# xcompact3d/x3d2

Measured on AMD Instinct MI355X. Metric: DoF*steps/s (whole node), TGV 512^3 per GPU, full fractional step, higher is better.
Workload: dtype f64; 1 GPU; TGV 512x512x512 all-periodic, Re=1600, dt=1e-3, RK3 (3 substeps/step), compact6/classic schemes, rocFFT Poisson (configs[2]); per_gpu=512^3, driver=fused, parallelism=domain decomposition 1x1x1, decomposition=yslabs, decomposition_requested=auto, poisson_z_first=228

## Files before the change

include/x3d2_hip.h:

```cpp
#ifndef X3D2_HIP_H
#define X3D2_HIP_H

#include <stddef.h>

#ifdef X3D_SINGLE_PREC
typedef float x3d_real;
#else
typedef double x3d_real;
#endif

#ifdef __cplusplus
extern "C" {
#endif

enum { X3D_DIR_X = 1, X3D_DIR_Y = 2, X3D_DIR_Z = 3, X3D_DIR_C = 4 };
enum { X3D_BC_PERIODIC = 0, X3D_BC_NEUMANN = 1, X3D_BC_DIRICHLET = 2, X3D_BC_HALO = -1 };
enum { X3D_X_FACE = 1100, X3D_Y_FACE = 1010, X3D_Z_FACE = 110 };
#define X3D_N_HALO 4

typedef struct x3d_backend x3d_backend;
typedef struct x3d_tdsops x3d_tdsops;
typedef struct x3d_poisson x3d_poisson;

const char *x3d_last_error(void);
// ... 231 lines not shown
int x3d_sfft010_set_waves(x3d_sfft010 *p, const x3d_real *waves, const x3d_real *ax, const x3d_real *bx, const x3d_real *ay,
                          const x3d_real *by, const x3d_real *az, const x3d_real *bz);
int x3d_sfft010_set_stretching(x3d_sfft010 *p, int sym, const x3d_real *a0, const x3d_real *a1);
int x3d_sfft010_periodicity_y(x3d_sfft010 *p, x3d_real *f_out, const x3d_real *f_in, int undo);
int x3d_sfft010_forward_local(x3d_sfft010 *p, const x3d_real *f_in, x3d_real *sendbuf);
int x3d_sfft010_fft_z(x3d_sfft010 *p, x3d_real *recvbuf, int dir);
int x3d_sfft010_postprocess_010(x3d_sfft010 *p, x3d_real *recvbuf);
int x3d_sfft010_backward_local(x3d_sfft010 *p, const x3d_real *sendbuf, x3d_real *f_out);

int x3d_poisson_zfirst_ok(x3d_poisson *p, int *ok);
int x3d_tds_pair_zfirst_ok(x3d_backend *b, const x3d_tdsops *ta, const x3d_tdsops *tb, int *ok);
int x3d_poisson_zfirst_middle(x3d_poisson *p);
int x3d_poisson_zfirst_forward(x3d_poisson *p, const x3d_real *f_in);
int x3d_poisson_zfirst_backward(x3d_poisson *p, x3d_real *f_out);
int x3d_poisson_solve_000_zfirst(x3d_poisson *p, x3d_real *f);
int x3d_poisson_set_stretching_zfirst(x3d_poisson *p, int sym, const x3d_real *a0, const x3d_real *a1);
int x3d_poisson_create_proxy(x3d_backend *b, x3d_poisson **out, x3d_real *spectrum, int ny, long px, int (*middle)(void *user),
                             void *user);
int x3d_poisson_solve_010_rows_zfirst(x3d_poisson *p, x3d_real *f);
int x3d_tds_pair_zfirst(x3d_backend *b, x3d_poisson *poisson, int mode, x3d_real *out1, x3d_real *out2, const x3d_real *in1,
                        const x3d_real *in2, const x3d_tdsops *ta, const x3d_tdsops *tb, int *done);

typedef struct x3d_sfftz x3d_sfftz;
int x3d_sfftz_create(x3d_backend *b, x3d_sfftz **out, const int nglob_cell[3], int py, int ry, int parts);
int x3d_sfftz_destroy(x3d_sfftz *p);
int x3d_sfftz_sizes(const x3d_sfftz *p, long out[16]);
int x3d_sfftz_spectrum(const x3d_sfftz *p, x3d_real **c, int *ny, long *px);
int x3d_sfftz_set_waves(x3d_sfftz *p, const x3d_real *rw, const x3d_real *ax, const x3d_real *bx, const x3d_real *ay,
                        const x3d_real *by, const x3d_real *az, const x3d_real *bz);
int x3d_sfftz_tds_pair(x3d_sfftz *p, int mode, x3d_real *out1, x3d_real *out2, const x3d_real *in1, const x3d_real *in2,
// ... 166 lines not shown
```

x3d2_amd/_lib.py:

```python
import ctypes
import os
import subprocess

from .common import X3dError

HERE = os.path.dirname(os.path.abspath(__file__))
SINGLE = os.environ.get("X3D_SINGLE_PREC") == "1"
LIB_PATH = os.path.join(HERE, "libx3d2_hip_sp.so" if SINGLE else "libx3d2_hip.so")
CSRC = os.path.join(HERE, "csrc")

REAL = ctypes.c_float if SINGLE else ctypes.c_double
NP_REAL = "float32" if SINGLE else "float64"
c_double_p = ctypes.POINTER(REAL)
c_int_p = ctypes.POINTER(ctypes.c_int)
VP = ctypes.c_void_p
I, D, SZT = ctypes.c_int, REAL, ctypes.c_size_t


def torch_real():
    import torch
    return torch.float32 if SINGLE else torch.float64

PROTOTYPES = {
    "x3d_last_error": (ctypes.c_char_p, []),
# ... 141 lines not shown
    "x3d_sfft010_postprocess_010_part": (I, [VP, VP, I]),
    "x3d_sfft010_destroy": (I, [VP]),
    "x3d_sfft010_sizes": (I, [VP, ctypes.POINTER(ctypes.c_long)]),
    "x3d_sfft010_set_waves": (I, [VP] + [c_double_p] * 7),
    "x3d_sfft010_set_stretching": (I, [VP, I, c_double_p, c_double_p]),
    "x3d_sfft010_periodicity_y": (I, [VP, VP, VP, I]),
    "x3d_sfft010_forward_local": (I, [VP, VP, VP]),
    "x3d_sfft010_fft_z": (I, [VP, VP, I]),
    "x3d_sfft010_postprocess_010": (I, [VP, VP]),
    "x3d_sfft010_backward_local": (I, [VP, VP, VP]),
    "x3d_poisson_zfirst_ok": (I, [VP, c_int_p]),
    "x3d_poisson_zfirst_middle": (I, [VP]),
    "x3d_poisson_zfirst_forward": (I, [VP, VP]),
    "x3d_poisson_zfirst_backward": (I, [VP, VP]),
    "x3d_poisson_solve_000_zfirst": (I, [VP, VP]),
    "x3d_tds_pair_zfirst": (I, [VP, VP, I, VP, VP, VP, VP, VP, VP, c_int_p]),
    "x3d_sfftz_create": (I, [VP, ctypes.POINTER(VP), c_int_p, I, I, I]),
    "x3d_sfftz_destroy": (I, [VP]),
    "x3d_sfftz_sizes": (I, [VP, ctypes.POINTER(ctypes.c_long)]),
    "x3d_sfftz_set_waves": (I, [VP] + [c_double_p] * 7),
    "x3d_sfftz_tds_pair": (I, [VP, I, VP, VP, VP, VP, VP, VP, c_int_p]),
    "x3d_sfftz_z": (I, [VP, VP, I]),
    "x3d_sfftz_z_field": (I, [VP, VP, I]),
    "x3d_sfftz_x_forward": (I, [VP, VP, I]),
    "x3d_sfftz_y_stage": (I, [VP, VP, I, I]),
    "x3d_sfftz_x_backward": (I, [VP, VP, I]),
    "x3d_sfftz_tds_pair_rows": (I, [VP, I, VP, VP, VP, VP, VP, VP, I, I, c_int_p]),
    "x3d_sfftz_z_rows": (I, [VP, VP, I, I, I]),
    "x3d_sfftz_x_forward_rows": (I, [VP, VP, I, I, I]),
    "x3d_sfftz_x_backward_rows": (I, [VP, VP, I, I, I]),
# ... 134 lines not shown
```

x3d2_amd/backend.py:

```python
import ctypes

import numpy as np
import torch

from . import _lib
from .common import (CELL, DIR_C, DIR_X, DIR_Y, DIR_Z, N_HALO, NULL_LOC, VERT, X_FACE, Y_FACE, Z_FACE, X3dError,
                     get_rdr_from_dirs, move_data_loc)
from .field import Allocator
from .parallel import Comm
from .switches import Switches
from .tdsops import Tdsops

VP = ctypes.c_void_p


def _dp(a):
    if a.dtype != np.dtype(_lib.NP_REAL):
        a = np.ascontiguousarray(a, dtype=_lib.NP_REAL)
    return a.ctypes.data_as(_lib.c_double_p)


class HipBackend:
    n_halo = N_HALO

# ... 615 lines not shown

    def zfirst_pairs_ok(self, t_a, t_b):
        flag = ctypes.c_int(0)
        _lib.check(self.lib.x3d_tds_pair_zfirst_ok(self.h, t_a.handle, t_b.handle, ctypes.byref(flag)))
        return bool(flag.value)

    def tds_apply_mean(self, du, u, tdsops, direction, mean_target):
        if u.data_loc == NULL_LOC:
            raise X3dError("You must set the data_loc before calling volume integral.")
        out = VP()
        ncell = float(np.prod(self.mesh.get_global_dims(CELL)))
        _lib.check(self.lib.x3d_tds_solve_mean(self.h, du.ptr, u.ptr, tdsops.handle, direction, self._dims(u.data_loc), ncell,
                                               float(mean_target), ctypes.byref(out)))
        return out

    def tds_apply(self, du, u, tdsops, direction, accumulate=False, scale=1.0):
        if not self._decomposed(direction):
            _lib.check(self.lib.x3d_tds_solve_acc(self.h, du.ptr, u.ptr, tdsops.handle, direction,
                                                  int(accumulate), float(scale)))
            return
        self._tds_dist(du, u, tdsops, direction, accumulate=accumulate, scale=scale)

    def tds_solve(self, du, u, tdsops):
        if u.dir != du.dir:
            raise X3dError("DIR mismatch between fields in tds_solve.")
        if u.data_loc != NULL_LOC:
            du.set_data_loc(move_data_loc(u.data_loc, u.dir, tdsops.move))
        direction = u.dir
        if direction == DIR_C:
            raise X3dError("tds_solve needs a directional field")
# ... 460 lines not shown
```

x3d2_amd/csrc/common.h:

```cpp
#pragma once
#include <hip/hip_runtime.h>

#include <cstdarg>
#include <cstdio>
#include <cstring>
#include <vector>

#include "../../include/x3d2_hip.h"

typedef x3d_real real_t;
#ifdef X3D_SINGLE_PREC
typedef float2 real2_t;
#define make_real2 make_float2
#else
typedef double2 real2_t;
#define make_real2 make_double2
#endif
#ifdef X3D_SINGLE_PREC
#define X3D_FFT_R2C HIPFFT_R2C
#define X3D_FFT_C2R HIPFFT_C2R
#define X3D_FFT_C2C HIPFFT_C2C
#define x3d_fftExecR2C hipfftExecR2C
#define x3d_fftExecC2R hipfftExecC2R
#define x3d_fftExecC2C hipfftExecC2C
// ... 70 lines not shown
    z = (z ^ (z >> 30)) * 0xBF58476D1CE4E5B9ull;
    z = (z ^ (z >> 27)) * 0x94D049BB133111EBull;
    return z ^ (z >> 31);
}

struct PencilGeom {
    int np;
    int dim0;
    long s0, s1, rs;
};

#define X3D_SW_UNSET (-0x7fffffffL - 1)
struct x3d_switches {
    long no_via_x, no_xscan, no_ygen, no_ytile, no_q5, no_direct, sfft010_split_xy;
    long no_circ, no_halo_circ, no_uniform, xscan_p1, no_ztile, no_tds_pair, no_npw2, no_tile3, xdir_generic, no_xcirc;
    long no_tds_lincomb, no_zfirst010, no_zfirst, no_xwide, no_xwide_upd;
    long no_spectral_pad, no_fft512, no_rwt, no_r2c512, no_y010, y010_no_db, no_onchip2, no_slab_fused_z;
    long lazy_dump, lazy_report, lazy_keep_zero_terms;
    long pad_x;
    long slab_z_split;
    long lazy_rules;
    long y010_form;
    long via_x;
    long ytile;
    long ygen;
    long x_fast;
    long x_tq3;
    long x_circ;
};
void x3d_switches_from_env(x3d_switches *sw);

// ... 213 lines not shown
```

x3d2_amd/csrc/poisson.hip:

```cpp
#include "fft_util.h"
#include "poisson_priv.h"
#include "spectral000.h"
int x3d_proxy_hook(x3d_poisson *p, int which, real_t *f);

__global__ void k_fill_pad(real_t *__restrict__ a, size_t rows, int nxm, int nxs, real_t v)
{
    const size_t r = (size_t)blockIdx.x * blockDim.x + threadIdx.x;
    if (r >= rows) return;
    for (int i = nxm; i < nxs; i++) a[r * nxs + i] = v;
}

static int upload_pitched(void *dst, const void *src, size_t rows, int nxm, int nxs, size_t elem)
{
    X3D_HIP(hipMemset(dst, 0, rows * nxs * elem));
    X3D_HIP(hipMemcpy2D(dst, nxs * elem, src, nxm * elem, nxm * elem, rows, hipMemcpyHostToDevice));
    return 0;
}

__global__ void __launch_bounds__(256)
    k_process_spectral_000(real2_t *__restrict__ c, const real_t *__restrict__ waves, int nxs, int ny, int nz,
                           int nx, const real_t *__restrict__ ax, const real_t *__restrict__ bx,
                           const real_t *__restrict__ ay, const real_t *__restrict__ by,
                           const real_t *__restrict__ az, const real_t *__restrict__ bz)
{
// ... 77 lines not shown
        p->r2c512 = p->nx == 512 && (batch % 2) == 0 && !b->sw.no_r2c512;
    }
    *out = p;
    return 0;
}

extern "C" int x3d_poisson_destroy(x3d_poisson *p)
{
    X3D_RANGE(__func__);
    if (!p) return 0;
    if (p->ext_middle) { delete p; return 0; }
    hipfftDestroy(p->plan_fw);
    hipfftDestroy(p->plan_bw);
    if (p->fast512) { hipfftDestroy(p->plan_x_fw); hipfftDestroy(p->plan_x_bw); }
    if (p->y010 == 1) { hipfftDestroy(p->plan_x010_fw); hipfftDestroy(p->plan_x010_bw); }
    hipFree(p->c); hipFree(p->waves); hipFree(p->ab); hipFree(p->work); hipFree(p->rwT); hipFree(p->rwZ);
    hipFree(p->lu[0]); hipFree(p->lu[1]); hipFree(p->luz[0]); hipFree(p->luz[1]);
    delete p;
    return 0;
}

static int x_forward_512(x3d_poisson *p, const real_t *f)
{
    ProfScope ps(p->b, X3D_K_FFT, 1);
    if (p->r2c512)
        return x3d_fft512_r2c(p->b, (real2_t *)p->c, f, (long)p->ny * p->nz, p->b->nxp, p->nxs);
    X3D_FFT(hipfftSetStream(p->plan_x_fw, p->b->stream));
    X3D_FFT(x3d_fftExecR2C(p->plan_x_fw, (x3d_fft_real *)f, (x3d_fft_cplx *)p->c));
    return 0;
}

// ... 422 lines not shown
```

x3d2_amd/csrc/poisson_priv.h:

```cpp
#pragma once
#include <hipfft/hipfft.h>

#include "common.h"

struct x3d_poisson {
    x3d_backend *b;
    int nx, ny, nz;
    int nxm, nxs;
    hipfftHandle plan_fw, plan_bw;
    real2_t *c;
    real_t *waves;
    real_t *rwT;
    real_t *ab;
    void *work;
    size_t work_size;
    int stretched, sym;
    real_t *lu[2];
    real_t *luz[2];
    size_t c_elems;
    int fast512;
    int r2c512;
    hipfftHandle plan_x_fw, plan_x_bw;
    int y010;
    hipfftHandle plan_x010_fw, plan_x010_bw;
    real_t *rwZ;
    int (*ext_middle)(void *user);
    void *ext_user;
    real2_t *ext_c;
    int ext_ny;
    long ext_px;
};
```

x3d2_amd/csrc/switches.hip:

```cpp
#include <cstdlib>

#include "common.h"

enum SwKind {
    SW_FLAG,
    SW_INT,
    SW_MASK,
    SW_FORM,
};
struct SwEntry {
    const char *name;
    SwKind kind;
    long unset;
    long x3d_switches::*field;
};
#define F(name, field) {name, SW_FLAG, 0, &x3d_switches::field}
static const SwEntry g_table[] = {
    F("X3D_NO_XSCAN", no_xscan),
    F("X3D_XDIR_GENERIC", xdir_generic),
    F("X3D_XSCAN_P1", xscan_p1),
    F("X3D_NO_TILE3", no_tile3),
    F("X3D_NO_XCIRC", no_xcirc),
    F("X3D_NO_CIRC", no_circ),
    F("X3D_NO_HALO_CIRC", no_halo_circ),
// ... 3 lines not shown
    F("X3D_NO_XWIDE_UPD", no_xwide_upd),
    F("X3D_NO_VIA_X", no_via_x),
    F("X3D_NO_YTILE", no_ytile),
    F("X3D_NO_ZTILE", no_ztile),
    F("X3D_NO_YGEN", no_ygen),
    F("X3D_NO_Q5", no_q5),
    F("X3D_NO_DIRECT", no_direct),
    F("X3D_NO_TDS_PAIR", no_tds_pair),
    F("X3D_NO_NPW2", no_npw2),
    F("X3D_NO_ONCHIP2", no_onchip2),
    F("X3D_NO_SPECTRAL_PAD", no_spectral_pad),
    F("X3D_NO_FFT512", no_fft512),
    F("X3D_NO_RWT", no_rwt),
    F("X3D_NO_R2C512", no_r2c512),
    F("X3D_NO_ZFIRST", no_zfirst),
    F("X3D_NO_ZFIRST010", no_zfirst010),
    F("X3D_NO_Y010", no_y010),
    F("X3D_Y010_NO_DB", y010_no_db),
    F("X3D_SFFT010_SPLIT_XY", sfft010_split_xy),
    F("X3D_NO_SLAB_FUSED_Z", no_slab_fused_z),
    F("X3D_LAZY_DUMP", lazy_dump),
    F("X3D_LAZY_REPORT", lazy_report),
    F("X3D_LAZY_KEEP_ZERO_TERMS", lazy_keep_zero_terms),
    {"X3D_LAZY_RULES", SW_MASK, 0xffffffffL, &x3d_switches::lazy_rules},
    {"X3D_PAD_X", SW_INT, X3D_SW_UNSET, &x3d_switches::pad_x},
    {"X3D_SLAB_Z_SPLIT", SW_INT, -1, &x3d_switches::slab_z_split},
    {"X3D_Y010_FORM", SW_FORM, 1, &x3d_switches::y010_form},
};
#undef F

// ... 34 lines not shown
```

x3d2_amd/csrc/tds.hip:

```cpp
#include "common.h"
#include "zfft_tile.h"

extern "C" int x3d_tdsops_create(x3d_backend *b, x3d_tdsops **out, int n_tds, int n_rhs, int move,
                                 int periodic, const real_t *coeffs, const real_t *coeffs_s,
                                 const real_t *coeffs_e, const real_t *dist_fw, const real_t *dist_bw,
                                 const real_t *dist_sa, const real_t *dist_sc, const real_t *dist_af,
                                 const real_t *stretch, const real_t *stretch_correct)
{
    X3D_RANGE(__func__);
    X3D_REQUIRE(b && out && coeffs && coeffs_s && coeffs_e && dist_fw && dist_bw && dist_sa && dist_sc &&
                    dist_af && stretch && stretch_correct,
                "x3d_tdsops_create: null argument");
    X3D_REQUIRE(n_rhs == n_tds || n_rhs == n_tds + 1, "x3d_tdsops_create: n_rhs must be n_tds or n_tds+1");
    X3D_REQUIRE(n_tds >= 8, "x3d_tdsops_create: n_tds=%d too small (the 4+4 boundary rows need n>=8)", n_tds);
    const int n = n_tds, nr = n_rhs, L = nr + 2;
    std::vector<real_t> h((size_t)10 * L + 81, 0.0);
    real_t *F = &h[0], *A = &h[L], *W = &h[2 * L], *Bw = &h[3 * L], *Sa = &h[4 * L], *Sc = &h[5 * L],
           *St = &h[6 * L], *Stc = &h[7 * L], *PF = &h[8 * L], *QB = &h[9 * L], *Cs = &h[10 * L];
    for (int j = 1; j <= nr; j++) {
        const bool real_row = j <= n;
        if (j <= 2) {
            F[j] = dist_af[j - 1];
            A[j] = 0.0;
        } else {
// ... 879 lines not shown
    if (int rc = check_len(b, t, dir, "tds_solve")) return rc;
    if (dir == X3D_DIR_X) return x3d_xdir_tds(b, du, u, t, accumulate, scale);
    if (!b->sw.no_onchip2) {
        bool done = false;
        if (int rc = x3d_onchip2_tds(b, du, u, t, dir, accumulate, scale, &done)) return rc;
        if (done) return 0;
    }
    if (!accumulate) {
        bool done = false;
        if (int rc = x3d_ygen_pair(b, dir, 2, du, nullptr, u, nullptr, t, t, &done)) return rc;
        if (done) return 0;
    }
    return x3d_generic_tds_local(b, du, u, t, dir, accumulate, scale);
}

int x3d_ytile_tds_pair(x3d_backend *b, int dir, int mode, real_t *out1, real_t *out2, const real_t *in1, const real_t *in2,
                       const x3d_tdsops *ta, const x3d_tdsops *tb, const TileHalo *halo, int other0, int nother,
                       bool *done);
int x3d_tds_halo_fix(x3d_backend *b, int dir, int mode, real_t *out1, real_t *out2, const real_t *brecv,
                     const x3d_tdsops *ta, const x3d_tdsops *tb);
int x3d_transeq_halo_fix_launch(x3d_backend *b, int dir, real_t *const r[3], const real_t *conv, real_t nu,
                                const real_t *brecv, const x3d_tdsops *der1st, const x3d_tdsops *der2nd);
int x3d_ytile_transeq3(x3d_backend *b, int dir, real_t *const r[3], const real_t *const f[3], real_t nu,
                       const x3d_tdsops *der1st, const x3d_tdsops *der1st_sym, const x3d_tdsops *der2nd,
                       const x3d_tdsops *der2nd_sym, int acc, const TileHalo *halo, int other0, int nother,
                       bool *done);

extern "C" int x3d_tds_solve_pair(x3d_backend *b, int dir, int mode, real_t *out1, real_t *out2, const real_t *in1,
                                  const real_t *in2, const x3d_tdsops *ta, const x3d_tdsops *tb)
{
// ... 672 lines not shown
```

x3d2_amd/csrc/xscan.hip:

```cpp
#include "common.h"


int npmax_of(const x3d_backend *b);

#include "xscan_core.h"
#include "zfft_tile.h"


template <bool ACC>
__device__ __forceinline__ void store_rows_q8(real_t *__restrict__ orow, int lane, const real_t (&r)[8],
                                              real_t scale)
{
    const int j = lane & 3;
    real_t a0 = r[0], a1 = r[1], b0 = r[2], b1 = r[3], c0 = r[4], c1 = r[5], d0 = r[6], d1 = r[7];
    rotl_pairs(a0, a1, b0, b1, c0, c1, d0, d1, j);
    b0 = dpp_quad(b0, 1); b1 = dpp_quad(b1, 1);
    c0 = dpp_quad(c0, 2); c1 = dpp_quad(c1, 2);
    d0 = dpp_quad(d0, 3); d1 = dpp_quad(d1, 3);
    rotl_pairs(a0, a1, b0, b1, c0, c1, d0, d1, j);
    real2_t *__restrict__ o2 = reinterpret_cast<real2_t *>(orow + (lane & ~3) * 8) + j;
    real2_t v0, v1, v2, v3;
    if (ACC) {
        v0 = o2[0]; v1 = o2[4]; v2 = o2[8]; v3 = o2[12];
        v0.x += scale * a0; v0.y += scale * a1;
// ... 111 lines not shown
        } else if (exact && n == nr) {
            real2_t *__restrict__ o2 = reinterpret_cast<real2_t *>(orow + lane * Q);
#pragma unroll
            for (int m = 0; m < Q / 2; m++) {
                real2_t v2;
                if (ACC) { v2 = o2[m]; v2.x += scale * r[2 * m]; v2.y += scale * r[2 * m + 1]; }
                else { v2.x = r[2 * m]; v2.y = r[2 * m + 1]; }
                o2[m] = v2;
            }
        } else {
#pragma unroll
            for (int q = 0; q < Q; q++) {
                const int j = first + q;
                if (j <= n) orow[j - 1] = ACC ? orow[j - 1] + scale * r[q] : r[q];
            }
        }
    }
}

template <int Q, bool NARROW, bool CIRC = false>
__global__ void __launch_bounds__(512) k_xscan_tds_lin(real_t *__restrict__ du, LinRows lr, XOp t, int np, long pitch,
                                                       CircOp co)
{
    extern __shared__ real_t lt[];
    if constexpr (!CIRC) {
        for (int i = threadIdx.x; i < LT_N(Q) * 64; i += blockDim.x) lt[i] = t.TL[i];
        __syncthreads();
    }
    int lane = threadIdx.x & 63;
    const int wave = __builtin_amdgcn_readfirstlane(threadIdx.x >> 6);
// ... 1187 lines not shown
                       (long)b->nxp, t->n_tds, SC_, t->circ)
#define PICK(Q_)                                                                                               \
    do {                                                                                                       \
        if (circ) { if (acc) LAUNCH(Q_, true, 3, scale); else LAUNCH(Q_, false, 3, 1.0); }                     \
        else if (fast && narrow) { if (acc) LAUNCH(Q_, true, 2, scale); else LAUNCH(Q_, false, 2, 1.0); }      \
        else if (fast) { if (acc) LAUNCH(Q_, true, 1, scale); else LAUNCH(Q_, false, 1, 1.0); }                \
        else { if (acc) LAUNCH(Q_, true, 0, scale); else LAUNCH(Q_, false, 0, 1.0); }                          \
    } while (0)
    if (Q == 8) PICK(8);
    else if (Q == 6) { if (acc) LAUNCH(6, true, 0, scale); else LAUNCH(6, false, 0, 1.0); }
    else PICK(4);
#undef PICK
#undef LAUNCH
    X3D_HIP(hipGetLastError());
    *done = true;
    return 0;
}

template <int Q, bool SAME, bool ACC, int FAST>
static int launch_transeq(x3d_backend *b, real_t *rhs, const real_t *u, const real_t *conv, real_t nu,
                          const x3d_tdsops *t1, const x3d_tdsops *t2, const x3d_tdsops *t3, int np, int blocks,
                          size_t lds, long pitch)
{
    X3D_LDS_OPTIN(b, (k_xscan_transeq<Q, SAME, ACC, FAST>));
    hipLaunchKernelGGL((k_xscan_transeq<Q, SAME, ACC, FAST>), dim3(blocks), dim3(FAST ? 1024 : 512), lds, b->stream, rhs, u, conv, xop_of(t1),
                       xop_of(t2), xop_of(t3), np, pitch, nu);
    X3D_HIP(hipGetLastError());
    return 0;
}

// ... 499 lines not shown
```

x3d2_amd/csrc/zfirst.hip:

```cpp
#include <vector>

#include "fft_util.h"
#include "poisson_priv.h"
#include "zfft_tile.h"

#define ZH_PX 520

int x3d_ztile_fft_run(x3d_backend *b, real_t *f, const ZfArg &zf, bool fwd, int y0, int nyr);

__global__ void __launch_bounds__(256)
    k_zh_rw(real_t *__restrict__ rwZ, const real_t *__restrict__ waves, int nx, int ny, int nxs)
{
    __shared__ real_t t[32][33];
    const int kz = blockIdx.z, x0 = blockIdx.x * 32, y0 = blockIdx.y * 32;
    const int tx = threadIdx.x & 31, ty = threadIdx.x >> 5;
    for (int r = ty; r < 32; r += 8) {
        const int x = x0 + tx, y = y0 + r, xm = x <= nx / 2 ? x : nx - x;
        const real_t wv = waves[((size_t)kz * ny + y) * nxs + xm];
        t[r][tx] = wv < 1.e-16 ? 0.0 : -1.0 / wv;
    }
    __syncthreads();
    for (int r = ty; r < 32; r += 8) rwZ[((size_t)kz * nx + x0 + r) * ny + y0 + tx] = t[tx][r];
}

template <int S>
__global__ void __launch_bounds__(512)
    k_c2c512_x(real2_t *__restrict__ c, const real2_t *__restrict__ twg, long nrows, long pitch)
{
    extern __shared__ real2_t zx[];
    real2_t *__restrict__ tws = zx + 8 * FP;
    if (threadIdx.x < 256) tws[threadIdx.x] = twg[threadIdx.x];
    __syncthreads();
    const int l = threadIdx.x & 63, w = __builtin_amdgcn_readfirstlane(threadIdx.x >> 6);
    real2_t *__restrict__ pen = zx + w * FP;
    long row = (long)blockIdx.x * 8 + w;
    const long step = (long)gridDim.x * 8;
    real2_t a[8], nx8[8];
    if (row < nrows) {
#pragma unroll
        for (int k = 0; k < 8; k++) nx8[k] = c[row * pitch + l + 64 * k];
    }
    for (; row < nrows; row += step) {
#pragma unroll
        for (int k = 0; k < 8; k++) a[k] = nx8[k];
        if (row + step < nrows) {
#pragma unroll
            for (int k = 0; k < 8; k++) nx8[k] = c[(row + step) * pitch + l + 64 * k];
        }
        fft512_wave<S>(a, pen, tws, l);
#pragma unroll
        for (int k = 0; k < 8; k++) c[row * pitch + l + 64 * k] = a[k];
    }
}

template <int S>
__global__ void __launch_bounds__(512)
    k_c2c1024_x(real2_t *__restrict__ c, const real2_t *__restrict__ twg, const real2_t *__restrict__ tw1024, long nrows,
                long pitch)
{
    extern __shared__ real2_t zx[];
    real2_t *__restrict__ tws = zx + 8 * FP;
    if (threadIdx.x < 256) tws[threadIdx.x] = twg[threadIdx.x];
// ... 103 lines not shown
    if (p->ext_middle) {
        if (int rc = x3d_fft512_init()) return rc;
        if (out) *out = ZfArg{p->ext_c, x3d_fft512_twiddles(), p->ext_ny, p->ext_px, 0};
        *ok = !p->b->sw.no_zfirst;
        return 0;
    }
    if (p->b->sw.no_zfirst) return 0;
    if (!p->b->sw.no_zfirst010 && zfirst010_sizes(p)) {
        if (int rc = x3d_fft512_init()) return rc;
        if (int rc = fft1024_init()) return rc;
        if (out) *out = ZfArg{p->c, x3d_fft512_twiddles(), p->ny, (long)ZH010_PX, p->ny};
        *ok = true;
        return 0;
    }
    if (!zfirst_sizes(p)) return 0;
    if (!p->rwZ) {
        X3D_HIP(hipMalloc(&p->rwZ, sizeof(real_t) * 257 * 512 * 512));
        hipLaunchKernelGGL(k_zh_rw, dim3(16, 16, 257), dim3(256), 0, p->b->stream, p->rwZ, p->waves, p->nx, p->ny, p->nxs);
        X3D_HIP(hipGetLastError());
    }
    if (out) *out = ZfArg{p->c, x3d_fft512_twiddles(), p->ny, (long)ZH_PX};
    *ok = true;
    return 0;
}

bool x3d_zfirst_on_offer(x3d_poisson *p)
{
    return p && !p->b->sw.no_zfirst && (p->ext_middle != nullptr || zfirst_sizes(p));
}

extern "C" int x3d_poisson_zfirst_ok(x3d_poisson *p, int *ok)
{
    X3D_RANGE(__func__);
    X3D_REQUIRE(p && ok, "x3d_poisson_zfirst_ok: null argument");
    bool o = false;
    if (int rc = x3d_zfirst_arg(p, nullptr, &o)) return rc;
    *ok = o ? 1 : 0;
    return 0;
}

template <int S>
static int c2c_x(x3d_poisson *p, int kz0, int nkz)
{
    const int lds = sizeof(real2_t) * (8 * FP + 256);
    X3D_LDS_OPTIN(p->b, (k_c2c512_x<S>));
    const long nrows = (long)nkz * p->ny;
    long blocks = (nrows + 7) / 8;
    if (blocks > 2048) blocks = 2048;
    ProfScope ps(p->b, X3D_K_FFT, S < 0 ? 1 : 2);
    hipLaunchKernelGGL((k_c2c512_x<S>), dim3((unsigned)blocks), dim3(512), lds, p->b->stream,
                       p->c + (long)kz0 * p->ny * ZH_PX, x3d_fft512_twiddles(), nrows, (long)ZH_PX);
    X3D_HIP(hipGetLastError());
    return 0;
}

extern "C" int x3d_poisson_zfirst_middle(x3d_poisson *p)
{
    X3D_RANGE(__func__);
    X3D_REQUIRE(p, "x3d_poisson_zfirst_middle: null argument");
    bool ok = false;
    if (int rc = x3d_zfirst_arg(p, nullptr, &ok)) return rc;
    X3D_REQUIRE(ok || p->ext_middle, "x3d_poisson_zfirst_middle: not a 512^3 all-periodic solver (x3d_poisson_zfirst_ok)");
    X3D_LAZY_EAGER(p->b);
    if (p->ext_middle) return p->ext_middle(p->ext_user);
    if (p->stretched) {
        x3d_backend *b = p->b;
        const int lds = sizeof(real2_t) * (8 * FP + 256);
        const long nrows = 257L * p->ny;
// ... 10 lines not shown
            ProfScope ps(b, X3D_K_SPECTRAL);
            if (int rc = x3d_y010_run(b, p->c, ZH010_PX, p->nx, p->ny, p->nz, 3, p->ab, p->sym, p->luz, &done, 257)) return rc;
            X3D_REQUIRE(done, "x3d_poisson_zfirst_middle: y pass refused");
        }
        {
            ProfScope ps(b, X3D_K_SPECTRAL);
            if (int rc = x3d_y010_run(b, p->c, ZH010_PX, p->nx, p->ny, p->nz, 4, p->ab, p->sym, p->luz, &done, 257)) return rc;
            X3D_REQUIRE(done, "x3d_poisson_zfirst_middle: y pass refused");
        }
        ProfScope ps(b, X3D_K_FFT, 2);
        hipLaunchKernelGGL((k_c2c1024_x<1>), dim3(blocks), dim3(512), lds, b->stream, p->c, x3d_fft512_twiddles(), g_tw1024,
                           nrows, (long)ZH010_PX);
        X3D_HIP(hipGetLastError());
        return 0;
    }
    if (int rc = c2c_x<-1>(p, 0, 257)) return rc;
    if (int rc = x3d_fft512_run_zh(p->b, p->c, ZH_PX, 0, 257, p->rwZ, p->ab, p->nx, p->ny, p->nz)) return rc;
    return c2c_x<1>(p, 0, 257);
}

extern "C" int x3d_poisson_create_proxy(x3d_backend *b, x3d_poisson **out, x3d_real *spectrum, int ny, long px,
                                        int (*middle)(void *), void *user)
{
    X3D_RANGE(__func__);
    X3D_REQUIRE(b && out && spectrum && middle && ny > 0 && px >= b->nx, "x3d_poisson_create_proxy: bad argument");
    X3D_REQUIRE(b->nz == 512 && b->nx % 16 == 0 && ny <= b->ny, "x3d_poisson_create_proxy: 512-row z pencils");
    x3d_poisson *p = new x3d_poisson();
    memset(p, 0, sizeof *p);
    p->b = b;
    p->nx = b->nx; p->ny = ny; p->nz = 512;
    p->ext_middle = middle; p->ext_user = user;
    p->ext_c = reinterpret_cast<real2_t *>(spectrum); p->ext_ny = ny; p->ext_px = px;
    if (int rc = x3d_fft512_init()) return rc;
// ... 78 lines not shown
```

x3d2_amd/poisson_fft.py:

```python
import ctypes
import math

import numpy as np

from . import _lib
from .common import CELL, X3dError

VP = ctypes.c_void_p


def wave_numbers(n, L, d, periodic, c_a, c_b, c_alpha):
    pi = 4.0 * math.atan(1.0)
    i = np.arange(1, n + 1, dtype=np.float64)
    if periodic:
        a, b = np.sin((i - 1) * pi / n), np.cos((i - 1) * pi / n)
    else:
        a, b = np.sin((i - 1) * pi / 2 / n), np.cos((i - 1) * pi / 2 / n)
    k, e, k2 = np.zeros(n), np.zeros(n), np.zeros(n)

    def mod_wave(w):
        wp = c_a * 2 * d * np.sin(0.5 * w) + c_b * 2 * d * np.sin(1.5 * w)
        return wp / (1.0 + 2 * c_alpha * np.cos(w))

    if periodic:
# ... 305 lines not shown
        self.undo_periodicity_y(f, temp)

    def solve_poisson(self, f, temp):
        self.poisson(f, temp)

    def zfirst_ok(self):
        if type(self) is not HipPoissonFFT or self.case not in ("000", "010") or getattr(self.backend, "lazy", False):
            return False
        ok = ctypes.c_int(0)
        _lib.check(self.backend.lib.x3d_poisson_zfirst_ok(self.h, ctypes.byref(ok)))
        return bool(ok.value)

    def zfirst_middle(self):
        _lib.check(self.backend.lib.x3d_poisson_zfirst_middle(self.h))

    def zfirst_forward(self, f):
        _lib.check(self.backend.lib.x3d_poisson_zfirst_forward(self.h, f.ptr))

    def zfirst_backward(self, f):
        _lib.check(self.backend.lib.x3d_poisson_zfirst_backward(self.h, f.ptr))

    def solve_zfirst(self, f):
        _lib.check(self.backend.lib.x3d_poisson_solve_000_zfirst(self.h, f.ptr))

    def interleaved_rows(self):
        if type(self) is HipPoissonFFT and self.case == "010" and self.ny_glob % 2 == 0:
            return self.ny_glob
        return 0

    def solve_interleaved(self, f):
# ... 677 lines not shown
```

x3d2_amd/solver.py:

```python
import numpy as np

from .common import (BC_DIRICHLET, BC_NEUMANN, CELL, DIR_C, DIR_X, DIR_Y, DIR_Z, RDR_C2Z, RDR_X2Y, RDR_X2Z,
                     RDR_Y2Z, RDR_Z2C, RDR_Z2X, VERT, Y_FACE, X3dError)
from .tdsops import Dirps
from .time_integrator import TimeIntegrator
from .vector_calculus import VectorCalculus


class SolverConfig:

    def __init__(self, Re=1600.0, dt=1e-3, n_iters=10, n_output=0, time_intg="RK3", poisson_solver_type="FFT",
                 der1st_scheme="compact6", der2nd_scheme="compact6", interpl_scheme="classic",
                 stagder_scheme="compact6", lowmem_transeq=False, fused=False, n_species=0, pr_species=None,
                 ibm_on=False):
        self.Re, self.dt, self.n_iters, self.n_output = Re, dt, n_iters, n_output
        self.time_intg, self.poisson_solver_type = time_intg, poisson_solver_type
        self.der1st_scheme, self.der2nd_scheme = der1st_scheme, der2nd_scheme
        self.interpl_scheme, self.stagder_scheme = interpl_scheme, stagder_scheme
        self.lowmem_transeq = lowmem_transeq
        self.n_species = int(n_species)
        self.pr_species = [1.0] * self.n_species if pr_species is None else [float(x) for x in pr_species]
        self.fused = fused
        self.ibm_on = bool(ibm_on)

# ... 64 lines not shown
            raise X3dError('poisson_solver_type is not valid. Use "FFT" or "CG".')
        self.pending_grad = None
        ns = self.time_integrator.nstage
        e = self.sw.epi3_stages
        self._epi3_stages = {int(v) for v in e.split(",")} if e else set(range(1, ns + 1))
        self.n_epi3 = 0
        self.rot_request, self.rot_applied = 0.0, False
        self.n_rot_fused = self.n_interleaved = 0
        self.n_zfirst = 0
        pf = backend.poisson_fft if cfg.poisson_solver_type == "FFT" else None
        self._zfirst = bool(pf is not None and getattr(pf, "zfirst_ok", lambda: False)())
        if self._zfirst:
            z = self.zdirps
            self._zfirst = (backend.zfirst_pairs_ok(z.interpl_v2p, z.stagder_v2p)
                            and backend.zfirst_pairs_ok(z.interpl_p2v, z.stagder_p2v))
        self.shift_request = None
        self.pending_walls = None
        self.mean_request, self._mean_ready, self.n_mean_taken = None, None, 0
        backend.before_read.append(self.flush_grad)
        self.lowmem_transeq = bool(getattr(cfg, "lowmem_transeq", False))
        if self.fused:
            self.transeq = self.transeq_fused
        else:
            self.transeq = self.transeq_lowmem if self.lowmem_transeq else self.transeq_default
        if self.fused:
            self.pressure_correction = self.pressure_correction_fused
        self.ibm = None
        self.les = None
        self.keep_pressure, self.pressure, self.pressure_wanted = False, None, False

# ... 194 lines not shown
        for d, dp, o0, no in second:
            b.transeq_planes(d, du, dv, dw, u, v, w, nu, dp, True, o0, no)
        for d, dp in slow:
            b.transeq_dir(d, du, dv, dw, u, v, w, nu, dp, accumulate=True)
        for d, dp in halo:
            b.transeq_halo_finish(d, du, dv, dw, u, v, w, nu, dp, hb[d])

    def pressure_correction_fused(self, u, v, w, defer_grad=False):
        b, al = self.backend, self.backend.allocator
        x, y, z = self.xdirps, self.ydirps, self.zdirps
        t1, t2, t3, a1, a2 = (al.get_block(DIR_X) for _ in range(5))
        upd = self.time_integrator.pending_update
        walls, self.pending_walls = self.pending_walls or (None, None, None), None
        mean, self.mean_request, self._mean_ready = self.mean_request, None, None
        want_p = self.keep_pressure and self.pressure_wanted
        for out, fld, op, wall in ((t1, u, x.stagder_v2p, walls[0]), (t2, v, x.interpl_v2p, walls[1]),
                                   (t3, w, x.interpl_v2p, walls[2])):
            spec = upd.pop(fld.data.data_ptr(), None)
            take_mean = fld is u and mean is not None and defer_grad and b.comm.size == 1 and not b._decomposed(DIR_X)
            if spec is None:
                if wall is not None:
                    b.field_set_face_from_field(fld, wall, 0.0, Y_FACE)
                if take_mean:
                    sh = b.tds_apply_mean(out, fld, op, DIR_X, mean)
                    self._mean_ready = (u.data.data_ptr(), float(mean), sh, b.red_epoch)
                else:
                    b.tds_apply(out, fld, op, DIR_X)
            elif take_mean:
                sh = b.tds_lincomb(out, op, DIR_X, *spec, wall=wall, mean_target=mean)
                self._mean_ready = (u.data.data_ptr(), float(mean), sh, b.red_epoch)
            else:
                b.tds_lincomb(out, op, DIR_X, *spec, wall=wall)
# ... 10 lines not shown
            if self._zfirst_solve(a1, a2, t2, t3):
                b.tds_jobs(DIR_Y, [(1, a1, a2, t2, None, y.interpl_p2v, y.stagder_p2v),
                                   (2, t1, None, t3, None, y.interpl_p2v, None)])
                return self._finish_pressure_correction(u, v, w, (t1, t2, t3, a1, a2), defer_grad)
            b.tds_jobs(DIR_Z, jz)
        elif b._decomposed(DIR_Y) or b._decomposed(DIR_Z):
            nil = nil if nil and not want_p and self._zpairs_interleave(nil, jz[0]) else 0
            if nil:
                jz = [(0, t2, None, a1, a2, z.interpl_v2p, z.stagder_v2p)]
                div = t2
                self.n_interleaved += 1
            self._div_grad_decomposed(jy, jz, forward=True, nil=nil)
        else:
            b.tds_pair(*jy[0], DIR_Y)
            b.tds_apply(a2, t3, y.interpl_v2p, DIR_Y)
            if self._zfirst and not want_p and self._zfirst_solve(a1, a2, t2, t3):
                b.tds_pair(1, a1, a2, t2, None, y.interpl_p2v, y.stagder_p2v, DIR_Y)
                b.tds_apply(t1, t3, y.interpl_p2v, DIR_Y)
                return self._finish_pressure_correction(u, v, w, (t1, t2, t3, a1, a2), defer_grad)
            if nil and not want_p and b.tds_pair_yperm(0, t2, None, a1, a2, z.interpl_v2p, z.stagder_v2p, nil):
                div = t2
                self.n_interleaved += 1
            else:
                nil = 0
                b.tds_pair(*jz[0], DIR_Z)
        p = div
        if nil:
            b.poisson_fft.solve_interleaved(p)
        elif self.cfg.poisson_solver_type == "FFT":
            b.poisson_fft.solve_poisson(p, t2)
        else:
# ... 14 lines not shown
            b.tds_pair(1, a1, a2, t1, None, y.interpl_p2v, y.stagder_p2v, DIR_Y)
            b.tds_apply(t2, t3, y.interpl_p2v, DIR_Y)
            t1, t2 = t2, t1
        else:
            jz = [(1, t2, t3, p, None, z.interpl_p2v, z.stagder_p2v)]
            jy = [(1, a1, a2, t2, None, y.interpl_p2v, y.stagder_p2v),
                  (2, t1, None, t3, None, y.interpl_p2v, None)]
            if b._decomposed(DIR_Y) or b._decomposed(DIR_Z):
                self._div_grad_decomposed(jy, jz, forward=False)
            else:
                b.tds_pair(*jz[0], DIR_Z)
                b.tds_pair(*jy[0], DIR_Y)
                b.tds_apply(t1, t3, y.interpl_p2v, DIR_Y)
        self._finish_pressure_correction(u, v, w, (t1, t2, t3, a1, a2), defer_grad)

    def _zfirst_solve(self, a1, a2, t2, t3):
        b, z = self.backend, self.zdirps
        pipe = getattr(b.poisson_fft, "zfirst_solve_pipelined", None)
        if pipe is not None and not b._decomposed(DIR_Z) and \
                pipe(a1, a2, t2, t3, z.interpl_v2p, z.stagder_v2p, z.interpl_p2v, z.stagder_p2v):
            self.n_zfirst += 1
            return True
        if not b.tds_pair_zfirst(0, None, None, a1, a2, z.interpl_v2p, z.stagder_v2p):
            return False
        b.poisson_fft.zfirst_middle()
        if not b.tds_pair_zfirst(1, t2, t3, None, None, z.interpl_p2v, z.stagder_p2v):
            raise X3dError("pressure_correction: the z-first pair served the divergence but not the gradient")
        self.n_zfirst += 1
        return True

    def _finish_pressure_correction(self, u, v, w, blocks, defer_grad):
        al = self.backend.allocator
# ... 139 lines not shown
```

Measured before the change: 3.383 billion DoF*steps/s.

## Fuse x-direction compact divergence with forward real FFT in pressure solve

Adds a kernel that applies the x-direction compact operator and then immediately does a packed 512-point real-to-complex FFT along x, writing spectral rows. Because the operands arrive already x-transformed, the Poisson middle stage can skip its forward c2c x-FFT, and the inverse x-FFT untangles the packed layout. The goal is to remove one full-field read/write pass and one FFT launch per substep. It adds a second 512^3 wave table and a path that only works for uniform periodic 512 grids on a single GPU, gated by several conditions including the absence of a pipelined zfirst solver.

```diff
diff --git a/include/x3d2_hip.h b/include/x3d2_hip.h
--- a/include/x3d2_hip.h
+++ b/include/x3d2_hip.h
@@ -269,6 +269,11 @@
 int x3d_poisson_zfirst_forward(x3d_poisson *p, const x3d_real *f_in);
 int x3d_poisson_zfirst_backward(x3d_poisson *p, x3d_real *f_out);
 int x3d_poisson_solve_000_zfirst(x3d_poisson *p, x3d_real *f);
+int x3d_tds_solve_xfft_ok(x3d_backend *b, const x3d_tdsops *t, int *ok);
+int x3d_tds_solve_xfft(x3d_backend *b, x3d_real *du, const x3d_real *u, const x3d_tdsops *t);
+int x3d_poisson_xfft_ok(x3d_poisson *p, int *ok);
+int x3d_poisson_zfirst_middle_xpacked(x3d_poisson *p);
+int x3d_c2c512_x_rows(x3d_backend *b, x3d_real *c, long nrows, long pitch, int mode);
 int x3d_poisson_set_stretching_zfirst(x3d_poisson *p, int sym, const x3d_real *a0, const x3d_real *a1);
 int x3d_poisson_create_proxy(x3d_backend *b, x3d_poisson **out, x3d_real *spectrum, int ny, long px, int (*middle)(void *user),
                              void *user);
diff --git a/x3d2_amd/_lib.py b/x3d2_amd/_lib.py
--- a/x3d2_amd/_lib.py
+++ b/x3d2_amd/_lib.py
@@ -179,6 +179,11 @@
     "x3d_poisson_zfirst_forward": (I, [VP, VP]),
     "x3d_poisson_zfirst_backward": (I, [VP, VP]),
     "x3d_poisson_solve_000_zfirst": (I, [VP, VP]),
+    "x3d_tds_solve_xfft_ok": (I, [VP, VP, c_int_p]),
+    "x3d_tds_solve_xfft": (I, [VP, VP, VP, VP]),
+    "x3d_poisson_xfft_ok": (I, [VP, c_int_p]),
+    "x3d_poisson_zfirst_middle_xpacked": (I, [VP]),
+    "x3d_c2c512_x_rows": (I, [VP, VP, ctypes.c_long, ctypes.c_long, I]),
     "x3d_tds_pair_zfirst": (I, [VP, VP, I, VP, VP, VP, VP, VP, VP, c_int_p]),
     "x3d_sfftz_create": (I, [VP, ctypes.POINTER(VP), c_int_p, I, I, I]),
     "x3d_sfftz_destroy": (I, [VP]),
diff --git a/x3d2_amd/backend.py b/x3d2_amd/backend.py
--- a/x3d2_amd/backend.py
+++ b/x3d2_amd/backend.py
@@ -653,6 +653,16 @@
                                                float(mean_target), ctypes.byref(out)))
         return out
 
+    def tds_apply_xfft_ok(self, tdsops):
+        if self._decomposed(DIR_X):
+            return False
+        flag = ctypes.c_int(0)
+        _lib.check(self.lib.x3d_tds_solve_xfft_ok(self.h, tdsops.handle, ctypes.byref(flag)))
+        return bool(flag.value)
+
+    def tds_apply_xfft(self, du, u, tdsops):
+        _lib.check(self.lib.x3d_tds_solve_xfft(self.h, du.ptr, u.ptr, tdsops.handle))
+
     def tds_apply(self, du, u, tdsops, direction, accumulate=False, scale=1.0):
         if not self._decomposed(direction):
             _lib.check(self.lib.x3d_tds_solve_acc(self.h, du.ptr, u.ptr, tdsops.handle, direction,
diff --git a/x3d2_amd/csrc/common.h b/x3d2_amd/csrc/common.h
--- a/x3d2_amd/csrc/common.h
+++ b/x3d2_amd/csrc/common.h
@@ -108,7 +108,7 @@
 struct x3d_switches {
     long no_via_x, no_xscan, no_ygen, no_ytile, no_q5, no_direct, sfft010_split_xy;
     long no_circ, no_halo_circ, no_uniform, xscan_p1, no_ztile, no_tds_pair, no_npw2, no_tile3, xdir_generic, no_xcirc;
-    long no_tds_lincomb, no_zfirst010, no_zfirst, no_xwide, no_xwide_upd;
+    long no_tds_lincomb, no_zfirst010, no_zfirst, no_xwide, no_xwide_upd, no_xfft_div;
     long no_spectral_pad, no_fft512, no_rwt, no_r2c512, no_y010, y010_no_db, no_onchip2, no_slab_fused_z;
     long lazy_dump, lazy_report, lazy_keep_zero_terms;
     long pad_x;
diff --git a/x3d2_amd/csrc/poisson.hip b/x3d2_amd/csrc/poisson.hip
--- a/x3d2_amd/csrc/poisson.hip
+++ b/x3d2_amd/csrc/poisson.hip
@@ -115,7 +115,7 @@
     hipfftDestroy(p->plan_bw);
     if (p->fast512) { hipfftDestroy(p->plan_x_fw); hipfftDestroy(p->plan_x_bw); }
     if (p->y010 == 1) { hipfftDestroy(p->plan_x010_fw); hipfftDestroy(p->plan_x010_bw); }
-    hipFree(p->c); hipFree(p->waves); hipFree(p->ab); hipFree(p->work); hipFree(p->rwT); hipFree(p->rwZ);
+    hipFree(p->c); hipFree(p->waves); hipFree(p->ab); hipFree(p->work); hipFree(p->rwT); hipFree(p->rwZ); hipFree(p->rwZp);
     hipFree(p->lu[0]); hipFree(p->lu[1]); hipFree(p->luz[0]); hipFree(p->luz[1]);
     delete p;
     return 0;
diff --git a/x3d2_amd/csrc/poisson_priv.h b/x3d2_amd/csrc/poisson_priv.h
--- a/x3d2_amd/csrc/poisson_priv.h
+++ b/x3d2_amd/csrc/poisson_priv.h
@@ -24,6 +24,7 @@
     int y010;
     hipfftHandle plan_x010_fw, plan_x010_bw;
     real_t *rwZ;
+    real_t *rwZp;
     int (*ext_middle)(void *user);
     void *ext_user;
     real2_t *ext_c;
diff --git a/x3d2_amd/csrc/switches.hip b/x3d2_amd/csrc/switches.hip
--- a/x3d2_amd/csrc/switches.hip
+++ b/x3d2_amd/csrc/switches.hip
@@ -41,6 +41,7 @@
     F("X3D_NO_RWT", no_rwt),
     F("X3D_NO_R2C512", no_r2c512),
     F("X3D_NO_ZFIRST", no_zfirst),
+    F("X3D_NO_XFFT_DIV", no_xfft_div),
     F("X3D_NO_ZFIRST010", no_zfirst010),
     F("X3D_NO_Y010", no_y010),
     F("X3D_Y010_NO_DB", y010_no_db),
diff --git a/x3d2_amd/csrc/tds.hip b/x3d2_amd/csrc/tds.hip
--- a/x3d2_amd/csrc/tds.hip
+++ b/x3d2_amd/csrc/tds.hip
@@ -917,6 +917,26 @@
     return x3d_generic_tds_local(b, du, u, t, dir, accumulate, scale);
 }
 
+bool x3d_xscan_tds_xfft_ok(const x3d_backend *b, const x3d_tdsops *t);
+int x3d_xscan_tds_xfft(x3d_backend *b, real_t *du, const real_t *u, const x3d_tdsops *t);
+extern "C" int x3d_tds_solve_xfft_ok(x3d_backend *b, const x3d_tdsops *t, int *ok)
+{
+    X3D_RANGE(__func__);
+    X3D_REQUIRE(b && t && ok, "x3d_tds_solve_xfft_ok: null argument");
+    *ok = x3d_xscan_tds_xfft_ok(b, t) ? 1 : 0;
+    return 0;
+}
+extern "C" int x3d_tds_solve_xfft(x3d_backend *b, real_t *du, const real_t *u, const x3d_tdsops *t)
+{
+    X3D_RANGE(__func__);
+    if (b) X3D_LAZY_SYNC(b);
+    X3D_LAZY_EAGER(b);
+    X3D_REQUIRE(b && du && u && t, "x3d_tds_solve_xfft: null argument");
+    X3D_REQUIRE(du != u, "x3d_tds_solve_xfft: du and u must be distinct blocks");
+    if (int rc = check_len(b, t, X3D_DIR_X, "tds_solve_xfft")) return rc;
+    return x3d_xscan_tds_xfft(b, du, u, t);
+}
+
 int x3d_ytile_tds_pair(x3d_backend *b, int dir, int mode, real_t *out1, real_t *out2, const real_t *in1, const real_t *in2,
                        const x3d_tdsops *ta, const x3d_tdsops *tb, const TileHalo *halo, int other0, int nother,
                        bool *done);
diff --git a/x3d2_amd/csrc/xscan.hip b/x3d2_amd/csrc/xscan.hip
--- a/x3d2_amd/csrc/xscan.hip
+++ b/x3d2_amd/csrc/xscan.hip
@@ -149,6 +149,54 @@
                 const int j = first + q;
                 if (j <= n) orow[j - 1] = ACC ? orow[j - 1] + scale * r[q] : r[q];
             }
+        }
+    }
+}
+
+__global__ void __launch_bounds__(512, 4) k_xscan_tds_xfft(real_t *__restrict__ du, const real_t *__restrict__ u, int np,
+                                                           long pitch, CircOp co, const real2_t *__restrict__ twg)
+{
+    constexpr int Q = 8;
+    extern __shared__ real2_t xf[];
+    real2_t *__restrict__ tws = xf + 8 * FP256;
+    if (threadIdx.x < 256) tws[threadIdx.x] = twg[threadIdx.x];
+    __syncthreads();
+    const int lane = threadIdx.x & 63;
+    const int wave = __builtin_amdgcn_readfirstlane(threadIdx.x >> 6);
+    real2_t *__restrict__ pen = xf + wave * FP256;
+    const int nwaves = gridDim.x * (blockDim.x >> 6);
+    const int p0 = blockIdx.x * (blockDim.x >> 6) + wave;
+    const int wsw = (lane >> 2) & 3, rsw = (lane >> 4) & 3;
+    real_t nb[Q];
+    if (p0 < np) load_body<Q>(nb, u + (long)p0 * pitch, lane);
+    for (int p = p0; p < np; p += nwaves) {
+        real_t w[Q + 8], r[Q];
+        window_from_body<Q>(w, nb, lane);
+        if (p + nwaves < np) load_body<Q>(nb, u + (long)(p + nwaves) * pitch, lane);
+        circ_solve<Q, true>(w, r, co, lane);
+        wave_lds_fence();
+#pragma unroll
+        for (int q = 0; q < 4; q++) pen[4 * lane + (q ^ wsw)] = make_real2(r[2 * q], r[2 * q + 1]);
+        wave_lds_fence();
+        real2_t a[4], c[4];
+#pragma unroll
+        for (int k = 0; k < 4; k++) a[k] = pen[64 * k + ((lane & ~3) | ((lane & 3) ^ rsw))];
+        fft256_wave<-1>(a, pen, tws, lane);
+#pragma unroll
+        for (int f = 0; f < 4; f++) pen[lane + 64 * f] = a[f];
+        wave_lds_fence();
+#pragma unroll
+        for (int f = 0; f < 4; f++) c[f] = pen[(256 - lane - 64 * f) & 255];
+        real2_t *__restrict__ o2 = reinterpret_cast<real2_t *>(du + (long)p * pitch);
+#pragma unroll
+        for (int f = 0; f < 4; f++) {
+            const int k = lane + 64 * f;
+            const real2_t wk = twiddle<-1>(tws, k);
+            const real_t er = 0.5 * (a[f].x + c[f].x), ei = 0.5 * (a[f].y - c[f].y);
+            const real_t dr = 0.5 * (a[f].y + c[f].y), di = 0.5 * (c[f].x - a[f].x);
+            real2_t F = make_real2(er + (wk.x * dr - wk.y * di), ei + (wk.x * di + wk.y * dr));
+            if (f == 0 && lane == 0) F = make_real2(a[0].x + a[0].y, a[0].x - a[0].y);
+            o2[k] = F;
         }
     }
 }
@@ -1366,6 +1414,29 @@
 #undef LAUNCH
     X3D_HIP(hipGetLastError());
     *done = true;
+    return 0;
+}
+
+int x3d_fft512_init();
+const real2_t *x3d_fft512_twiddles();
+bool x3d_xscan_tds_xfft_ok(const x3d_backend *b, const x3d_tdsops *t)
+{
+    return sizeof(real_t) == 8 && b->sw.x_fast && !b->sw.no_xfft_div && b->nx == 512 && b->nxp % 2 == 0 && xscan_ok(t) && t->tab.Q == 8 &&
+           t->tab.bulk_only && t->n_tds == 512 && t->tab.n_rhs == 512 && stencil_narrow(t) && t->uniform && t->circ_ok &&
+           !b->sw.no_circ;
+}
+int x3d_xscan_tds_xfft(x3d_backend *b, real_t *du, const real_t *u, const x3d_tdsops *t)
+{
+    X3D_REQUIRE(x3d_xscan_tds_xfft_ok(b, t), "x3d_tds_solve_xfft: not on offer for this operator (x3d_tds_solve_xfft_ok)");
+    if (int rc = x3d_fft512_init()) return rc;
+    const int np = b->ny * b->nz;
+    const size_t lds = sizeof(real2_t) * (8 * FP256 + 256);
+    int blocks = (np + 7) / 8;
+    blocks = blocks > 1024 ? 1024 : blocks;
+    ProfScope ps(b, X3D_K_TDS_FWD, X3D_DIR_X);
+    hipLaunchKernelGGL(k_xscan_tds_xfft, dim3(blocks), dim3(512), lds, b->stream, du, u, np, (long)b->nxp, t->circ,
+                       x3d_fft512_twiddles());
+    X3D_HIP(hipGetLastError());
     return 0;
 }
 
diff --git a/x3d2_amd/csrc/zfirst.hip b/x3d2_amd/csrc/zfirst.hip
--- a/x3d2_amd/csrc/zfirst.hip
+++ b/x3d2_amd/csrc/zfirst.hip
@@ -9,13 +9,14 @@
 int x3d_ztile_fft_run(x3d_backend *b, real_t *f, const ZfArg &zf, bool fwd, int y0, int nyr);
 
 __global__ void __launch_bounds__(256)
-    k_zh_rw(real_t *__restrict__ rwZ, const real_t *__restrict__ waves, int nx, int ny, int nxs)
+    k_zh_rw(real_t *__restrict__ rwZ, const real_t *__restrict__ waves, int nx, int ny, int nxs, int packed)
 {
     __shared__ real_t t[32][33];
     const int kz = blockIdx.z, x0 = blockIdx.x * 32, y0 = blockIdx.y * 32;
     const int tx = threadIdx.x & 31, ty = threadIdx.x >> 5;
     for (int r = ty; r < 32; r += 8) {
-        const int x = x0 + tx, y = y0 + r, xm = x <= nx / 2 ? x : nx - x;
+        const int x = x0 + tx, y = y0 + r;
+        const int xm = packed ? (x < 2 ? x * (nx / 2) : x >> 1) : (x <= nx / 2 ? x : nx - x);
         const real_t wv = waves[((size_t)kz * ny + y) * nxs + xm];
         t[r][tx] = wv < 1.e-16 ? 0.0 : -1.0 / wv;
     }
@@ -23,10 +24,11 @@
     for (int r = ty; r < 32; r += 8) rwZ[((size_t)kz * nx + x0 + r) * ny + y0 + tx] = t[tx][r];
 }
 
-template <int S>
+template <int S, bool UNT = false>
 __global__ void __launch_bounds__(512)
     k_c2c512_x(real2_t *__restrict__ c, const real2_t *__restrict__ twg, long nrows, long pitch)
 {
+    static_assert(!UNT || S > 0, "the untangle belongs to the inverse transform");
     extern __shared__ real2_t zx[];
     real2_t *__restrict__ tws = zx + 8 * FP;
     if (threadIdx.x < 256) tws[threadIdx.x] = twg[threadIdx.x];
@@ -36,16 +38,31 @@
     long row = (long)blockIdx.x * 8 + w;
     const long step = (long)gridDim.x * 8;
     real2_t a[8], nx8[8];
+    auto col = [&](int k) { return UNT ? 2 * (l + 64 * (k >> 1)) + (k & 1) : l + 64 * k; };
     if (row < nrows) {
 #pragma unroll
-        for (int k = 0; k < 8; k++) nx8[k] = c[row * pitch + l + 64 * k];
+        for (int k = 0; k < 8; k++) nx8[k] = c[row * pitch + col(k)];
     }
     for (; row < nrows; row += step) {
-#pragma unroll
-        for (int k = 0; k < 8; k++) a[k] = nx8[k];
+        if (UNT) {
+            wave_lds_fence();
+#pragma unroll
+            for (int j = 0; j < 4; j++) {
+                const real2_t A = nx8[2 * j], B = nx8[2 * j + 1];
+                const int m = l + 64 * j;
+                a[j] = m ? make_real2(A.x - B.y, A.y + B.x) : A;
+                pen[m ? 512 - m : 256] = m ? make_real2(A.x + B.y, A.y - B.x) : B;
+            }
+            wave_lds_fence();
+#pragma unroll
+            for (int k = 4; k < 8; k++) a[k] = pen[l + 64 * k];
+        } else {
+#pragma unroll
+            for (int k = 0; k < 8; k++) a[k] = nx8[k];
+        }
         if (row + step < nrows) {
 #pragma unroll
-            for (int k = 0; k < 8; k++) nx8[k] = c[(row + step) * pitch + l + 64 * k];
+            for (int k = 0; k < 8; k++) nx8[k] = c[(row + step) * pitch + col(k)];
         }
         fft512_wave<S>(a, pen, tws, l);
 #pragma unroll
@@ -179,13 +196,22 @@
         return 0;
     }
     if (!zfirst_sizes(p)) return 0;
-    if (!p->rwZ) {
-        X3D_HIP(hipMalloc(&p->rwZ, sizeof(real_t) * 257 * 512 * 512));
-        hipLaunchKernelGGL(k_zh_rw, dim3(16, 16, 257), dim3(256), 0, p->b->stream, p->rwZ, p->waves, p->nx, p->ny, p->nxs);
-        X3D_HIP(hipGetLastError());
-    }
+    if (int rc = x3d_fft512_init()) return rc;
     if (out) *out = ZfArg{p->c, x3d_fft512_twiddles(), p->ny, (long)ZH_PX};
     *ok = true;
+    return 0;
+}
+
+static int zh_table(x3d_poisson *p, bool packed, const real_t **out)
+{
+    real_t *&tab = packed ? p->rwZp : p->rwZ;
+    if (!tab) {
+        X3D_HIP(hipMalloc(&tab, sizeof(real_t) * 257 * 512 * 512));
+        hipLaunchKernelGGL(k_zh_rw, dim3(16, 16, 257), dim3(256), 0, p->b->stream, tab, p->waves, p->nx, p->ny, p->nxs,
+                           packed ? 1 : 0);
+        X3D_HIP(hipGetLastError());
+    }
+    *out = tab;
     return 0;
 }
 
@@ -204,19 +230,35 @@
     return 0;
 }
 
-template <int S>
-static int c2c_x(x3d_poisson *p, int kz0, int nkz)
+template <int S, bool UNT = false>
+static int c2c_x_rows(x3d_backend *b, real2_t *c, long nrows, long pitch)
 {
     const int lds = sizeof(real2_t) * (8 * FP + 256);
-    X3D_LDS_OPTIN(p->b, (k_c2c512_x<S>));
-    const long nrows = (long)nkz * p->ny;
+    X3D_LDS_OPTIN(b, (k_c2c512_x<S, UNT>));
     long blocks = (nrows + 7) / 8;
     if (blocks > 2048) blocks = 2048;
-    ProfScope ps(p->b, X3D_K_FFT, S < 0 ? 1 : 2);
-    hipLaunchKernelGGL((k_c2c512_x<S>), dim3((unsigned)blocks), dim3(512), lds, p->b->stream,
-                       p->c + (long)kz0 * p->ny * ZH_PX, x3d_fft512_twiddles(), nrows, (long)ZH_PX);
+    ProfScope ps(b, X3D_K_FFT, S < 0 ? 1 : 2);
+    hipLaunchKernelGGL((k_c2c512_x<S, UNT>), dim3((unsigned)blocks), dim3(512), lds, b->stream, c, x3d_fft512_twiddles(), nrows,
+                       pitch);
     X3D_HIP(hipGetLastError());
     return 0;
+}
+template <int S, bool UNT = false>
+static int c2c_x(x3d_poisson *p, int kz0, int nkz)
+{
+    return c2c_x_rows<S, UNT>(p->b, p->c + (long)kz0 * p->ny * ZH_PX, (long)nkz * p->ny, (long)ZH_PX);
+}
+
+extern "C" int x3d_c2c512_x_rows(x3d_backend *b, x3d_real *c, long nrows, long pitch, int mode)
+{
+    X3D_RANGE(__func__);
+    X3D_REQUIRE(b && c && nrows > 0 && pitch >= 512, "x3d_c2c512_x_rows: bad argument");
+    X3D_REQUIRE(mode == -1 || mode == 1 || mode == 2, "x3d_c2c512_x_rows: mode %d", mode);
+    X3D_LAZY_SYNC(b);
+    if (int rc = x3d_fft512_init()) return rc;
+    real2_t *c2 = reinterpret_cast<real2_t *>(c);
+    if (mode == -1) return c2c_x_rows<-1>(b, c2, nrows, pitch);
+    return mode == 1 ? c2c_x_rows<1>(b, c2, nrows, pitch) : c2c_x_rows<1, true>(b, c2, nrows, pitch);
 }
 
 extern "C" int x3d_poisson_zfirst_middle(x3d_poisson *p)
@@ -257,9 +299,36 @@
         X3D_HIP(hipGetLastError());
         return 0;
     }
+    const real_t *rw;
+    if (int rc = zh_table(p, false, &rw)) return rc;
     if (int rc = c2c_x<-1>(p, 0, 257)) return rc;
-    if (int rc = x3d_fft512_run_zh(p->b, p->c, ZH_PX, 0, 257, p->rwZ, p->ab, p->nx, p->ny, p->nz)) return rc;
+    if (int rc = x3d_fft512_run_zh(p->b, p->c, ZH_PX, 0, 257, rw, p->ab, p->nx, p->ny, p->nz)) return rc;
     return c2c_x<1>(p, 0, 257);
+}
+
+extern "C" int x3d_poisson_xfft_ok(x3d_poisson *p, int *ok)
+{
+    X3D_RANGE(__func__);
+    X3D_REQUIRE(p && ok, "x3d_poisson_xfft_ok: null argument");
+    *ok = 0;
+    if (p->ext_middle || p->stretched || p->b->sw.no_xfft_div) return 0;
+    bool o = false;
+    if (int rc = x3d_zfirst_arg(p, nullptr, &o)) return rc;
+    *ok = o ? 1 : 0;
+    return 0;
+}
+extern "C" int x3d_poisson_zfirst_middle_xpacked(x3d_poisson *p)
+{
+    X3D_RANGE(__func__);
+    X3D_REQUIRE(p, "x3d_poisson_zfirst_middle_xpacked: null argument");
+    int ok = 0;
+    if (int rc = x3d_poisson_xfft_ok(p, &ok)) return rc;
+    X3D_REQUIRE(ok, "x3d_poisson_zfirst_middle_xpacked: not on offer for this solver (x3d_poisson_xfft_ok)");
+    X3D_LAZY_EAGER(p->b);
+    const real_t *rw;
+    if (int rc = zh_table(p, true, &rw)) return rc;
+    if (int rc = x3d_fft512_run_zh(p->b, p->c, ZH_PX, 0, 257, rw, p->ab, p->nx, p->ny, p->nz)) return rc;
+    return c2c_x<1, true>(p, 0, 257);
 }
 
 extern "C" int x3d_poisson_create_proxy(x3d_backend *b, x3d_poisson **out, x3d_real *spectrum, int ny, long px,
diff --git a/x3d2_amd/poisson_fft.py b/x3d2_amd/poisson_fft.py
--- a/x3d2_amd/poisson_fft.py
+++ b/x3d2_amd/poisson_fft.py
@@ -343,6 +343,16 @@
     def zfirst_middle(self):
         _lib.check(self.backend.lib.x3d_poisson_zfirst_middle(self.h))
 
+    def xfft_ok(self):
+        if not self.zfirst_ok() or self.case != "000":
+            return False
+        ok = ctypes.c_int(0)
+        _lib.check(self.backend.lib.x3d_poisson_xfft_ok(self.h, ctypes.byref(ok)))
+        return bool(ok.value)
+
+    def zfirst_middle_xpacked(self):
+        _lib.check(self.backend.lib.x3d_poisson_zfirst_middle_xpacked(self.h))
+
     def zfirst_forward(self, f):
         _lib.check(self.backend.lib.x3d_poisson_zfirst_forward(self.h, f.ptr))
 
diff --git a/x3d2_amd/solver.py b/x3d2_amd/solver.py
--- a/x3d2_amd/solver.py
+++ b/x3d2_amd/solver.py
@@ -102,6 +102,12 @@
             z = self.zdirps
             self._zfirst = (backend.zfirst_pairs_ok(z.interpl_v2p, z.stagder_v2p)
                             and backend.zfirst_pairs_ok(z.interpl_p2v, z.stagder_p2v))
+        x = self.xdirps
+        self._xfft_div = bool(self._zfirst and getattr(pf, "xfft_ok", lambda: False)()
+                              and not hasattr(pf, "zfirst_solve_pipelined") and backend.comm.size == 1
+                              and not any(backend._decomposed(d) for d in (DIR_X, DIR_Y, DIR_Z))
+                              and backend.tds_apply_xfft_ok(x.stagder_v2p) and backend.tds_apply_xfft_ok(x.interpl_v2p))
+        self.n_xfft_div = 0
         self.shift_request = None
         self.pending_walls = None
         self.mean_request, self._mean_ready, self.n_mean_taken = None, None, 0
@@ -326,8 +332,15 @@
         walls, self.pending_walls = self.pending_walls or (None, None, None), None
         mean, self.mean_request, self._mean_ready = self.mean_request, None, None
         want_p = self.keep_pressure and self.pressure_wanted
+        xfft = self._xfft_div and not want_p and mean is None and all(wl is None for wl in walls)
         for out, fld, op, wall in ((t1, u, x.stagder_v2p, walls[0]), (t2, v, x.interpl_v2p, walls[1]),
                                    (t3, w, x.interpl_v2p, walls[2])):
+            if xfft:
+                spec = upd.pop(fld.data.data_ptr(), None)
+                if spec is not None:
+                    b.lincomb(*spec)
+                b.tds_apply_xfft(out, fld if spec is None else spec[0], op)
+                continue
             spec = upd.pop(fld.data.data_ptr(), None)
             take_mean = fld is u and mean is not None and defer_grad and b.comm.size == 1 and not b._decomposed(DIR_X)
             if spec is None:
@@ -368,7 +381,7 @@
         else:
             b.tds_pair(*jy[0], DIR_Y)
             b.tds_apply(a2, t3, y.interpl_v2p, DIR_Y)
-            if self._zfirst and not want_p and self._zfirst_solve(a1, a2, t2, t3):
+            if self._zfirst and not want_p and self._zfirst_solve(a1, a2, t2, t3, xpacked=xfft):
                 b.tds_pair(1, a1, a2, t2, None, y.interpl_p2v, y.stagder_p2v, DIR_Y)
                 b.tds_apply(t1, t3, y.interpl_p2v, DIR_Y)
                 return self._finish_pressure_correction(u, v, w, (t1, t2, t3, a1, a2), defer_grad)
@@ -413,8 +426,17 @@
                 b.tds_apply(t1, t3, y.interpl_p2v, DIR_Y)
         self._finish_pressure_correction(u, v, w, (t1, t2, t3, a1, a2), defer_grad)
 
-    def _zfirst_solve(self, a1, a2, t2, t3):
+    def _zfirst_solve(self, a1, a2, t2, t3, xpacked=False):
         b, z = self.backend, self.zdirps
+        if xpacked:
+            if not b.tds_pair_zfirst(0, None, None, a1, a2, z.interpl_v2p, z.stagder_v2p):
+                raise X3dError("pressure_correction: x-transformed operands, but the z-first pair declined the divergence")
+            b.poisson_fft.zfirst_middle_xpacked()
+            if not b.tds_pair_zfirst(1, t2, t3, None, None, z.interpl_p2v, z.stagder_p2v):
+                raise X3dError("pressure_correction: the z-first pair served the divergence but not the gradient")
+            self.n_zfirst += 1
+            self.n_xfft_div += 1
+            return True
         pipe = getattr(b.poisson_fft, "zfirst_solve_pipelined", None)
         if pipe is not None and not b._decomposed(DIR_Z) and \
                 pipe(a1, a2, t2, t3, z.interpl_v2p, z.stagder_v2p, z.interpl_p2v, z.stagder_p2v):
```

After: 3.520 billion DoF*steps/s, median of 6. 4.0% higher.
